# liuzuxin/FSRL

Measured on NVIDIA H100. Metric: env-steps/sec (collect+update) SafetyCarCircle-v0 PPO-Lag, higher is better.
Workload: dtype f32

## Files before the change

### fsrl_b200/csrc/ppo_persist.cu

```cuda
#include "ppo_persist.cuh"
#include "arena.cuh"
#include "ppo_loss.cuh"
#include "wgmma.cuh"
#include <cstdlib>
#include <cmath>
#include <vector>

namespace fsrl {
namespace pp {

using namespace wg;

constexpr int WQ = 2;
constexpr int NEPI = 128 * WQ;
constexpr int TPB = NEPI + 32;
constexpr int C1 = 16 / WQ;
constexpr int C2 = 32 / WQ;
constexpr int RB = 64;
constexpr int MB = 256;
constexpr int KC = 32, NCH = 256 / KC;
constexpr int SLOT_BYTES = 32768, NSLOT = 4;
constexpr int A_CHUNK = 64 * KC * 4;
constexpr int ACC_LD = 68;
constexpr int OUTP = 8;
constexpr int H_ = 256;
constexpr int IMG = 65536;
enum { I_H1A_HI, I_H1A_LO, I_H1T_HI, I_H1T_LO, I_DZA_HI, I_DZA_LO, I_DZT_HI, I_DZT_LO, I_W2A_HI, I_W2A_LO, I_W2B_HI, I_W2B_LO, N_IMG };
constexpr int DB2P_OFF = N_IMG * IMG;
constexpr int DW3P_OFF = DB2P_OFF + 4 * H_;
constexpr int DB3P_OFF = DW3P_OFF + 4 * H_ * OUTP;
constexpr int MAXD = 40;
constexpr int NSMAX = (MAXD + 1) * 32 + 32 + 32 * OUTP + 16;
constexpr int SLICE_OFF = DB3P_OFF + 4 * 16;
constexpr int NET_WS = SLICE_OFF + 8 * NSMAX;
constexpr int SUMSQ_FLOATS = 128;
constexpr int FLAG_LINE = 32;
constexpr int F_A = 0, F_C = 1, F_PER_NET = 2;
constexpr int TILE_PK = (64 * 64 / NEPI + 2) / 3;
constexpr int TILE_FLOATS = TILE_PK * NEPI * 4;
constexpr int SLICE_PK = (NSMAX + 2) / 3;
constexpr int XG_PER_NET = 16 * TILE_FLOATS + 8 * SLICE_PK * 4;
constexpr int MAX_MB = 16384;
constexpr long long WAIT_CYCLES = 6000000000LL;

struct Args {
    fsrl_ppo_update_t u;
    int n_mb, slot0;
    long long adam_t0;
    float* ws;
    unsigned* flags;
    int* err;
    const float* adam_tab;
    long long* dbg;
    int dbg_step;
    unsigned dp_seq;
    int dp_direct;
};
constexpr int DBG_CH = 48;
constexpr int DBG_N = DBG_CH + 2 * 3 * NCH;
#define STAMP(i) do { if (P.dbg && t == P.dbg_step) P.dbg[(size_t)blockIdx.x * DBG_N + (i)] = clock64(); } while (0)

struct AdamS { float w1, b2, w2, rbc2s, eps, neg_step; };
__device__ __forceinline__ float adam_one(float p, float g, float& m, float& v, const AdamS& a) {
    m = m + a.w1 * (g - m);
    v = v * a.b2 + (a.w2 * g) * g;
    const float sq = v > 0.f ? v * rsqrtf(v) : 0.f;
    const float denom = fmaf(sq, a.rbc2s, a.eps);
    return p + __fdividef(a.neg_step * m, denom);
}

__device__ __forceinline__ void fail(int* err, int code) {
    *reinterpret_cast<volatile int*>(err) = code;
    __threadfence_system();
    asm volatile("trap;");
}
__device__ __forceinline__ uint32_t pk_hash(float x, float y, float z) {
    const uint32_t a = __float_as_uint(x), b = __float_as_uint(y), c = __float_as_uint(z);
    return a ^ __funnelshift_l(b, b, 11) ^ __funnelshift_l(c, c, 22);
}
__device__ __forceinline__ bool pk_ok(const float4& v, uint32_t tag) { return (__float_as_uint(v.w) ^ pk_hash(v.x, v.y, v.z)) == tag; }
__device__ __forceinline__ void st_packet(float* p, float x, float y, float z, uint32_t tag) {
    asm volatile("st.relaxed.sys.global.v4.f32 [%0], {%1,%2,%3,%4};" ::"l"(p), "f"(x), "f"(y), "f"(z), "f"(__uint_as_float(tag ^ pk_hash(x, y, z))) : "memory");
}
__device__ __forceinline__ float4 ld_packet(const float* p) {
    float4 v;
    asm volatile("ld.relaxed.sys.global.v4.f32 {%0,%1,%2,%3}, [%4];" : "=f"(v.x), "=f"(v.y), "=f"(v.z), "=f"(v.w) : "l"(p) : "memory");
    return v;
}

__device__ __noinline__ float3 dp_gather(const float* src, long long stride, int me, int world, uint32_t tag,
                                        float ox, float oy, float oz, int* err, int code) {
    const long long t0w = clock64();
    float ax = 0.f, ay = 0.f, az = 0.f;
    for (int r0 = 0; r0 < world; r0 += 4) {
        float4 v[4];
        bool ok;
        do {
            ok = true;
#pragma unroll
            for (int k = 0; k < 4; ++k)
                if (r0 + k < world && r0 + k != me) v[k] = ld_packet(src + (size_t)(r0 + k) * stride);
#pragma unroll
            for (int k = 0; k < 4; ++k)
                if (r0 + k < world && r0 + k != me) ok = ok && pk_ok(v[k], tag);
            if (!ok && clock64() - t0w > 4 * WAIT_CYCLES) fail(err, code);
        } while (!ok);
#pragma unroll
        for (int k = 0; k < 4; ++k) {
            if (r0 + k >= world) continue;
            if (r0 + k == me) { ax += ox; ay += oy; az += oz; }
            else { ax += v[k].x; ay += v[k].y; az += v[k].z; }
        }
    }
    return make_float3(ax, ay, az);
}
__device__ __noinline__ void dp_push_all(const float* const* xg, size_t off, int me, int world, float x, float y, float z, uint32_t tag) {
    for (int r = 0; r < world; ++r)
        if (r != me) st_packet(const_cast<float*>(xg[r]) + off, x, y, z, tag);
}

__device__ __forceinline__ uint32_t mapa_u32(uint32_t local_saddr, uint32_t rank) {
    uint32_t r;
    asm volatile("mapa.shared::cluster.u32 %0, %1, %2;" : "=r"(r) : "r"(local_saddr), "r"(rank));
    return r;
}
__device__ __forceinline__ void st_cluster4(uint32_t raddr, float4 v) {
    asm volatile("st.shared::cluster.v4.f32 [%0], {%1,%2,%3,%4};" ::"r"(raddr), "f"(v.x), "f"(v.y), "f"(v.z), "f"(v.w) : "memory");
}
__device__ __forceinline__ void st_async4(uint32_t raddr, float4 v, uint32_t rbar) {
    asm volatile("st.async.weak.shared::cluster.mbarrier::complete_tx::bytes.v4.f32 [%0], {%1,%2,%3,%4}, [%5];"
                 ::"r"(raddr), "f"(v.x), "f"(v.y), "f"(v.z), "f"(v.w), "r"(rbar) : "memory");
}
__device__ __forceinline__ float ld_cluster(uint32_t raddr) {
    float v;
    asm volatile("ld.shared::cluster.f32 %0, [%1];" : "=f"(v) : "r"(raddr) : "memory");
    return v;
}
__device__ __forceinline__ void mbar_arrive_release_cluster2(uint32_t raddr0, uint32_t raddr1) {
    asm volatile("fence.acq_rel.cluster;\n\t"
                 "mbarrier.arrive.relaxed.cluster.shared::cluster.b64 _, [%0];\n\t"
                 "mbarrier.arrive.relaxed.cluster.shared::cluster.b64 _, [%1];" ::"r"(raddr0), "r"(raddr1) : "memory");
}
__device__ __forceinline__ bool mbar_wait_cluster(uint64_t* bar, uint32_t parity, long long timeout_cycles) {
    const long long t0 = clock64();
    while (true) {
        uint32_t ok;
        asm volatile(
            "{\n\t.reg .pred p;\n\t"
            "mbarrier.try_wait.parity.acquire.cluster.shared::cta.b64 p, [%1], %2;\n\t"
            "selp.u32 %0, 1, 0, p;\n\t}"
            : "=r"(ok) : "r"(smem_u32(bar)), "r"(parity) : "memory");
        if (ok) return true;
        if (clock64() - t0 > timeout_cycles) return false;
    }
}
__device__ __forceinline__ void cluster_sync_all() {
    asm volatile("barrier.cluster.arrive.release.aligned;\n\tbarrier.cluster.wait.acquire.aligned;" ::: "memory");
}

__device__ __forceinline__ bool elect_one() {
    uint32_t pred = 0;
    asm volatile(
        "{\n\t.reg .b32 rx;\n\t.reg .pred px;\n\t"
        "elect.sync rx|px, 0xffffffff;\n\t"
        "selp.u32 %0, 1, 0, px;\n\t}"
        : "=r"(pred));
    return pred != 0;
}
__device__ __forceinline__ void epi_bar() { asm volatile("bar.sync 1, %0;" ::"n"(NEPI) : "memory"); }
__device__ __forceinline__ void prefetch_l2(const void* p) { asm volatile("prefetch.global.L2 [%0];" ::"l"(p)); }

template <int NC>
__device__ __forceinline__ void acc_ld(const float* accs, int row, int col, float (&v)[NC]) {
#pragma unroll
    for (int q = 0; q < NC / 4; ++q) {
        const float4 x = *reinterpret_cast<const float4*>(accs + row * ACC_LD + col + 4 * q);
        v[4 * q] = x.x; v[4 * q + 1] = x.y; v[4 * q + 2] = x.z; v[4 * q + 3] = x.w;
    }
}
template <int NC>
__device__ __forceinline__ void acc_st(float* accs, int row, int col, const float (&v)[NC]) {
#pragma unroll
    for (int q = 0; q < NC / 4; ++q)
        *reinterpret_cast<float4*>(accs + row * ACC_LD + col + 4 * q) = make_float4(v[4 * q], v[4 * q + 1], v[4 * q + 2], v[4 * q + 3]);
}

template <int N>
__device__ __forceinline__ void gemm_phase(const unsigned char* ring, unsigned& qq, uint64_t* bar_full, uint32_t empty_r,
                                           float (&dm)[N / 2], float (&dc)[N / 2], int* err, int code, int lane,
                                           const Args& P, int t, int g) {
#pragma unroll
    for (int e = 0; e < N / 2; ++e) dm[e] = dc[e] = 0.f;
    const uint32_t ring_a = smem_u32(ring);
    constexpr uint32_t b_lbo = 16 * N, b_chunk = N * KC * 4;
    for (int j = 0; j < NCH; ++j, ++qq) {
        const int s = qq % NSLOT;
        if (!mbar_wait(&bar_full[s], (qq / NSLOT) & 1, WAIT_CYCLES)) fail(err, code);
#ifdef FSRL_PPO_CHUNK_STAMPS
        if (P.dbg && t == P.dbg_step && threadIdx.x < 32) P.dbg[(size_t)blockIdx.x * DBG_N + DBG_CH + 3 * NCH * g + 2 * NCH + j] = clock64();
#endif
        __syncwarp();
        wgmma_fence();
        const uint32_t base = ring_a + (uint32_t)s * SLOT_BYTES;
        const uint64_t ah0 = smem_desc(base, 1024, 128), al0 = smem_desc(base + A_CHUNK, 1024, 128);
        const uint64_t bh0 = smem_desc(base + 2 * A_CHUNK, b_lbo, 128), bl0 = smem_desc(base + 2 * A_CHUNK + b_chunk, b_lbo, 128);
#pragma unroll
        for (int ks = 0; ks < KC / 8; ++ks) {
            const uint64_t ah = ah0 + ks * (2048 / 16), al = al0 + ks * (2048 / 16);
            const uint64_t bh = bh0 + ks * (2 * b_lbo / 16), bl = bl0 + ks * (2 * b_lbo / 16);
            if constexpr (N == 32) {
                mma_m64n32k8_tf32(dc, al, bh);
                mma_m64n32k8_tf32(dc, ah, bl);
                mma_m64n32k8_tf32(dm, ah, bh);
            } else {
                mma_m64n64k8_tf32(dc, al, bh);
                mma_m64n64k8_tf32(dc, ah, bl);
                mma_m64n64k8_tf32(dm, ah, bh);
            }
        }
        wgmma_commit();
        if (j > 0) {
            wgmma_wait<1>();
            __syncwarp();
            if (lane < 8) mbar_arrive_cluster(empty_r + 8 * ((qq - 1) % NSLOT));
        }
    }
    wgmma_wait<0>();
    reg_fence(dm); reg_fence(dc);
    __syncwarp();
    if (lane < 8) mbar_arrive_cluster(empty_r + 8 * ((qq - 1) % NSLOT));
}
template <int N>
__device__ __forceinline__ void stage_acc(float* accs, const float (&dm)[N / 2], const float (&dc)[N / 2], int wq, int sp,
                                          int lane) {
    if (wq == 0) {
        const int r = 16 * sp + (lane >> 2);
#pragma unroll
        for (int i = 0; i < N / 8; ++i) {
            const int c = 8 * i + 2 * (lane & 3);
            *reinterpret_cast<float2*>(accs + r * ACC_LD + c) = make_float2(dm[4 * i] + dc[4 * i], dm[4 * i + 1] + dc[4 * i + 1]);
            *reinterpret_cast<float2*>(accs + (r + 8) * ACC_LD + c) =
                make_float2(dm[4 * i + 2] + dc[4 * i + 2], dm[4 * i + 3] + dc[4 * i + 3]);
        }
    }
    asm volatile("bar.sync %0, 64;" ::"r"(2 + sp) : "memory");
}

__device__ __forceinline__ void copy_operand(unsigned char* dst, const float* src, uint32_t bytes, uint64_t* bar, int g, int i,
                                             uint16_t cta_mask) {
    if (g == 1) {
        bulk_g2s(dst, src, bytes, bar);
        bulk_g2s(dst + bytes, src + IMG, bytes, bar);
        return;
    }
    const uint32_t piece = 2 * bytes / g, off = i * piece, part = off / bytes, in = off % bytes;
    bulk_g2s_multicast(dst + off, src + (size_t)part * IMG + in / 4, piece, bar, cta_mask);
}

template <int NC, int W>
__device__ __forceinline__ void transposed_stage(float* scr, const float (&hi)[NC], const float (&lo)[NC], int row, int c0) {
    constexpr int LO = W * 65;
#pragma unroll
    for (int j = 0; j < NC; ++j) {
        scr[(c0 + j) * 65 + row] = hi[j];
        scr[LO + (c0 + j) * 65 + row] = lo[j];
    }
}
template <int W>
__device__ __forceinline__ void transposed_flush(const float* scr, int et, float* img_hi, int row_base, int col_base) {
    constexpr int LO = W * 65;
    const int col = et % W;
    constexpr int GPT = 16 / (NEPI / W);
    const int g0 = (et / W) * GPT;
    float* dst = img_hi + (size_t)(row_base >> 2) * 256 + (size_t)(col_base + col) * 4;
#pragma unroll
    for (int q = 0; q < GPT; ++q) {
        const int g = g0 + q;
        const float* sh = scr + col * 65 + 4 * g;
        *reinterpret_cast<float4*>(dst + (size_t)g * 256) = make_float4(sh[0], sh[1], sh[2], sh[3]);
        *reinterpret_cast<float4*>(dst + IMG + (size_t)g * 256) = make_float4(sh[LO], sh[LO + 1], sh[LO + 2], sh[LO + 3]);
    }
}
template <int NC, int W>
__device__ __forceinline__ void store_transposed(float* scr, const float (&hi)[NC], const float (&lo)[NC], int row, int c0,
                                                 int et, float* img_hi, int row_base, int col_base) {
    transposed_stage<NC, W>(scr, hi, lo, row, c0);
    epi_bar();
    transposed_flush<W>(scr, et, img_hi, row_base, col_base);
    epi_bar();
}

__device__ __forceinline__ float half_sum(float v) {
#pragma unroll
    for (int o = 8; o > 0; o >>= 1) v += __shfl_xor_sync(0xffffffffu, v, o);
    return v;
}

struct SliceMap {
    int w1, b2, w3, b3, n;
    __device__ __host__ SliceMap(int D) { w1 = 0; b2 = (D + 1) * 32; w3 = b2 + 32; b3 = w3 + 32 * OUTP; n = b3 + 16; }
};

struct DpCtx {
    const float* const* xg;
    long long region;
    int me, world;
    uint32_t tag;
    int* err;
    int direct;
};
__device__ __forceinline__ int dp_owner(int et, int q, int world) { return (int)((unsigned)((et >> 5) * TILE_PK + q) % (unsigned)world); }

__device__ __noinline__ void dp_tile_send(DpCtx d, size_t off, const float* accs, int trow, int cb2, int et) {
    float g[C2];
    acc_ld<C2>(accs, trow, cb2, g);
#pragma unroll
    for (int q = 0; q < TILE_PK; ++q) {
        const size_t o_q = (size_t)d.me * d.region + off + (size_t)q * NEPI * 4;
        const float x = g[3 * q], y = 3 * q + 1 < C2 ? g[3 * q + 1] : 0.f, z = 3 * q + 2 < C2 ? g[3 * q + 2] : 0.f;
        if (d.direct) {
            dp_push_all(d.xg, o_q, d.me, d.world, x, y, z, d.tag);
        } else {
            const int o = dp_owner(et, q, d.world);
            if (o != d.me) st_packet(const_cast<float*>(d.xg[o]) + o_q, x, y, z, d.tag);
        }
    }
}
__device__ __noinline__ void dp_tile_reduce(DpCtx d, size_t off, float* accs, int trow, int cb2, int et) {
    float g[C2];
    acc_ld<C2>(accs, trow, cb2, g);
    const float inv_world = 1.0f / (float)d.world;
    const float* loc = d.xg[d.me];
#pragma unroll
    for (int q = 0; q < TILE_PK; ++q) {
        if (dp_owner(et, q, d.world) != d.me) continue;
        const float3 s3 = dp_gather(loc + off + (size_t)q * NEPI * 4, d.region, d.me, d.world, d.tag, g[3 * q],
                                    3 * q + 1 < C2 ? g[3 * q + 1] : 0.f, 3 * q + 2 < C2 ? g[3 * q + 2] : 0.f, d.err, 41);
        const float ax = s3.x * inv_world, ay = s3.y * inv_world, az = s3.z * inv_world;
        dp_push_all(d.xg, (size_t)FSRL_P2P_MAX_RANKS * d.region + off + (size_t)q * NEPI * 4, d.me, d.world, ax, ay, az, d.tag);
        g[3 * q] = ax;
        if (3 * q + 1 < C2) g[3 * q + 1] = ay;
        if (3 * q + 2 < C2) g[3 * q + 2] = az;
    }
    acc_st<C2>(accs, trow, cb2, g);
}
__device__ __noinline__ float dp_tile_finish(DpCtx d, size_t off, float* accs, int trow, int cb2, int et) {
    float g[C2];
    const long long t0w = clock64();
    if (d.direct) {
        float own[C2];
        acc_ld<C2>(accs, trow, cb2, own);
#pragma unroll
        for (int jq = 0; jq < C2; ++jq) g[jq] = 0.f;
        for (int r = 0; r < d.world; ++r) {
            if (r == d.me) {
#pragma unroll
                for (int jq = 0; jq < C2; ++jq) g[jq] += own[jq];
                continue;
            }
            const float* src = d.xg[d.me] + (size_t)r * d.region + off;
            float4 v[TILE_PK];
            bool ok;
            do {
                ok = true;
#pragma unroll
                for (int q = 0; q < TILE_PK; ++q) v[q] = ld_packet(src + (size_t)q * NEPI * 4);
#pragma unroll
                for (int q = 0; q < TILE_PK; ++q) ok = ok && pk_ok(v[q], d.tag);
                if (!ok && clock64() - t0w > 4 * WAIT_CYCLES) fail(d.err, 42);
            } while (!ok);
#pragma unroll
            for (int q = 0; q < TILE_PK; ++q) {
// ... 44 lines not shown
                    sp_g[3 * i], 3 * i + 1 < n ? sp_g[3 * i + 1] : 0.f, 3 * i + 2 < n ? sp_g[3 * i + 2] : 0.f, d.tag);
    const float* loc = d.xg[d.me];
    for (int i = et; i < n3; i += NEPI) {
        const float3 s3 = dp_gather(loc + off_s + 4 * (size_t)i, d.region, d.me, d.world, d.tag, sp_g[3 * i],
                                    3 * i + 1 < n ? sp_g[3 * i + 1] : 0.f, 3 * i + 2 < n ? sp_g[3 * i + 2] : 0.f, d.err, 40);
        sp_g[3 * i] = s3.x * inv_world;
        if (3 * i + 1 < n) sp_g[3 * i + 1] = s3.y * inv_world;
        if (3 * i + 2 < n) sp_g[3 * i + 2] = s3.z * inv_world;
    }
}

__device__ __forceinline__ bool red_cta() { return ((blockIdx.x >> 3) & 3) == ((blockIdx.x & 7) >> 2); }

__device__ __noinline__ float dp_tail(DpCtx d, size_t off_t, size_t off_s, float* accs, float* sp_g, int n, int trow, int cb2,
                                      int et, bool tile, bool slice) {
    if (tile && !d.direct) dp_tile_reduce(d, off_t, accs, trow, cb2, et);
    if (slice) dp_slices(d, off_s, sp_g, n, et);
    __syncwarp();
    return tile ? dp_tile_finish(d, off_t, accs, trow, cb2, et) : 0.f;
}

template <bool DP>
__global__ void __launch_bounds__(TPB, 1) ppo_persist_kernel(const Args P) {
    extern __shared__ __align__(1024) unsigned char smem_raw[];
    __shared__ __align__(8) uint64_t bar_full[NSLOT], bar_empty[NSLOT], bar_b, bar_w1;
    __shared__ float s_red[4][320];
    __shared__ float s_misc[32];
    __shared__ AdamS s_adam;
    __shared__ const float* s_xg[2][FSRL_P2P_MAX_RANKS];
    const fsrl_ppo_update_t& u = P.u;
    const int tid = threadIdx.x, warp = tid >> 5, lane = tid & 31;
    const int net = blockIdx.x >> 5, c = blockIdx.x & 31, a = c >> 3, b = c & 7;
    const bool is_g2 = c < 16;
    const int ka = (c & 15) >> 2, q4 = c & 3;

    const int D = u.D, A = u.A, C = u.C, H = H_;
    const int out = (net == 0) ? A : 1;
    const int n_cta = 32 * u.n_nets;
    float* wsn = P.ws + (size_t)net * NET_WS;
    float* sumsq_g = P.ws + (size_t)u.n_nets * NET_WS;
    unsigned* fl_net = P.flags + (size_t)net * F_PER_NET * FLAG_LINE;
    unsigned* fl_d2 = P.flags + (size_t)u.n_nets * F_PER_NET * FLAG_LINE;
    unsigned char* ring = smem_raw;
    float* accs = reinterpret_cast<float*>(smem_raw + NSLOT * SLOT_BYTES);
    float* small = accs + 64 * ACC_LD;
    const SliceMap sm(D);
    float* sp_p = small;
    float* sp_m = small + sm.n;
    float* sp_v = small + 2 * sm.n;
    float* sp_g = small + 3 * sm.n;
    float* land = small + 4 * sm.n;

    if (tid == 0) {
        for (int i = 0; i < NSLOT; ++i) { mbar_init(&bar_full[i], 1); mbar_init(&bar_empty[i], 4 * 8); }
        mbar_init(&bar_b, 1);
        mbar_init(&bar_w1, 4);
        fence_mbar_init();
    }
    __syncthreads();
    if (DP && threadIdx.x < 2 * FSRL_P2P_MAX_RANKS) s_xg[threadIdx.x / FSRL_P2P_MAX_RANKS][threadIdx.x % FSRL_P2P_MAX_RANKS] = P.u.p2p_xg[threadIdx.x / FSRL_P2P_MAX_RANKS][threadIdx.x % FSRL_P2P_MAX_RANKS];
    if (DP) __syncthreads();
    cluster_sync_all();

    const long long pbase = u.net_off[net];
    const ArenaLayout L = arena_layout(D, H, out, 0);
    const long long o_w1 = pbase + L.w1, o_b1 = pbase + L.b1, o_w2 = pbase + L.w2, o_b2 = pbase + L.b2,
                    o_w3 = pbase + L.w3, o_b3 = pbase + L.b3, o_ls = pbase + L.extra;

    if (warp == NEPI / 32) {
        if (elect_one()) {
            unsigned qq = 0;
            for (int t = 0; t < P.n_mb; ++t) {
                if (!flag_wait_ge<true>(fl_net + F_A * FLAG_LINE, 32u * (t + 1), WAIT_CYCLES)) fail(P.err, 10);
                STAMP(12);
                fence_proxy_async_global();
#pragma unroll 1
                for (int j = 0; j < NCH; ++j, ++qq) {
                    const int s = qq % NSLOT;
                    if (!mbar_wait(&bar_empty[s], ((qq / NSLOT) & 1) ^ 1, WAIT_CYCLES)) fail(P.err, 11);
#ifdef FSRL_PPO_CHUNK_STAMPS
                    STAMP(DBG_CH + j);
#endif
                    unsigned char* dst = ring + (size_t)s * SLOT_BYTES;
                    mbar_expect_tx(&bar_full[s], 3 * A_CHUNK);
                    const size_t ao = (size_t)a * 16384 + (size_t)j * 64 * KC, bo = (size_t)b * 8192 + (size_t)j * 32 * KC;
                    copy_operand(dst, wsn + (size_t)I_H1A_HI * IMG + ao, A_CHUNK, &bar_full[s], 8, b, 0xff);
                    copy_operand(dst + 2 * A_CHUNK, wsn + (size_t)I_W2A_HI * IMG + bo, A_CHUNK / 2, &bar_full[s], 1, 0, 0);
#ifdef FSRL_PPO_CHUNK_STAMPS
                    STAMP(DBG_CH + NCH + j);
#endif
                }
                STAMP(13);
                if (!flag_wait_ge<true>(fl_net + F_C * FLAG_LINE, 32u * (t + 1), WAIT_CYCLES)) fail(P.err, 12);
                STAMP(14);
                fence_proxy_async_global();
                const int ia = is_g2 ? I_W2B_HI : I_DZT_HI, ib = is_g2 ? I_DZA_HI : I_H1T_HI;
                const int blk_a = is_g2 ? ka : q4, blk_b = is_g2 ? q4 : ka;
                const uint16_t m4 = (uint16_t)(0xfu << (b & 4)), m2 = (uint16_t)(0x11u << (b & 3));
#pragma unroll 1
                for (int j = 0; j < NCH; ++j, ++qq) {
                    const int s = qq % NSLOT;
                    if (!mbar_wait(&bar_empty[s], ((qq / NSLOT) & 1) ^ 1, WAIT_CYCLES)) fail(P.err, 13);
#ifdef FSRL_PPO_CHUNK_STAMPS
                    STAMP(DBG_CH + 3 * NCH + j);
#endif
                    unsigned char* dst = ring + (size_t)s * SLOT_BYTES;
                    mbar_expect_tx(&bar_full[s], 4 * A_CHUNK);
                    const size_t ao = (size_t)blk_a * 16384 + (size_t)j * 64 * KC, bo = (size_t)blk_b * 16384 + (size_t)j * 64 * KC;
                    copy_operand(dst, wsn + (size_t)ia * IMG + ao, A_CHUNK, &bar_full[s], is_g2 ? 4 : 2, is_g2 ? b & 3 : b >> 2, is_g2 ? m4 : m2);
                    copy_operand(dst + 2 * A_CHUNK, wsn + (size_t)ib * IMG + bo, A_CHUNK, &bar_full[s], is_g2 ? 2 : 4, is_g2 ? b >> 2 : b & 3, is_g2 ? m2 : m4);
#ifdef FSRL_PPO_CHUNK_STAMPS
                    STAMP(DBG_CH + 4 * NCH + j);
#endif
                }
            }
        }
    } else {
        const int et = tid;
        const int sp = warp & 3;
        const int wq = warp >> 2;
        const int r16 = lane & 15, half = lane >> 4;
        const int trow = 16 * sp + r16;
        const int cb1 = 16 * half + C1 * wq;
        const int cb2 = 32 * half + C2 * wq;
        unsigned qq = 0;
        const uint32_t empty_r = mapa_u32(smem_u32(bar_empty), lane < 8 ? lane : 0);
        float w2p[C2], w2m[C2], w2v[C2];
        const int world = DP ? u.world : 1;
        auto dp_ctx = [&](int t_) {
            DpCtx d;
            const unsigned long long id = (unsigned long long)(P.adam_t0 + t_ + 1);
            d.xg = s_xg[(int)(id & 1ULL)];
            d.region = (long long)u.n_nets * XG_PER_NET;
            d.me = u.p2p_rank; d.world = world;
            d.tag = (P.dp_seq << 16) | (uint32_t)((t_ + 1) & 0xffff);
            d.err = P.err;
            d.direct = P.dp_direct;
            return d;
        };

        for (int i = et; i < sm.n; i += NEPI) {
            long long src = -1;
            if (i < sm.b2) { const int d = i / 32, kk = i % 32; src = (d < D) ? o_w1 + (long long)d * H + 32 * b + kk : o_b1 + 32 * b + kk; }
            else if (i < sm.w3) src = o_b2 + 32 * b + (i - sm.b2);
            else if (i < sm.b3) { const int oo = (i - sm.w3) / OUTP, jj = (i - sm.w3) % OUTP; if (jj < out) src = o_w3 + (long long)(32 * b + oo) * out + jj; }
            else { const int jj = i - sm.b3; if (jj < out) src = o_b3 + jj; else if (net == 0 && jj >= 8 && jj < 8 + A) src = o_ls + (jj - 8); }
            sp_p[i] = src >= 0 ? u.theta[src] : 0.f;
            sp_m[i] = src >= 0 ? u.adam_m[src] : 0.f;
            sp_v[i] = src >= 0 ? u.adam_v[src] : 0.f;
            sp_g[i] = 0.f;
        }
        if (!is_g2) {
            const int o = 64 * q4 + trow;
#pragma unroll
            for (int j = 0; j < C2; ++j) {
                const long long idx = o_w2 + (long long)(64 * ka + cb2 + j) * H + o;
                w2p[j] = u.theta[idx]; w2m[j] = u.adam_m[idx]; w2v[j] = u.adam_v[idx];
            }
        } else {
#pragma unroll
            for (int j = 0; j < C2; ++j) w2p[j] = w2m[j] = w2v[j] = 0.f;
        }
        epi_bar();

        for (int t = 0; t < P.n_mb; ++t) {
            const long long row0 = (long long)t * MB;
            const int slot = P.slot0 + t;
            if (et == 0) {
                s_adam.w1 = (float)(1.0 - u.beta1); s_adam.b2 = (float)u.beta2; s_adam.w2 = (float)(1.0 - u.beta2);
                s_adam.rbc2s = __ldg(P.adam_tab + 2 * t); s_adam.eps = (float)u.adam_eps; s_adam.neg_step = __ldg(P.adam_tab + 2 * t + 1);
                STAMP(0);
                if (P.dbg && t == P.dbg_step) { long long gt; asm volatile("mov.u64 %0, %%globaltimer;" : "=l"(gt)); P.dbg[(size_t)blockIdx.x * DBG_N + 30] = gt; }
                if (P.dbg && t == P.dbg_step + 64) {
                    long long gt; asm volatile("mov.u64 %0, %%globaltimer;" : "=l"(gt));
                    P.dbg[(size_t)blockIdx.x * DBG_N + 31] = gt;
                    P.dbg[(size_t)blockIdx.x * DBG_N + 29] = clock64();
                }
            }
            if (t + 1 < P.n_mb && et < 64) {
                const long long r = row0 + MB + 64 * a + et;
                prefetch_l2(u.obs + r * D);
                if (D > 32) prefetch_l2(u.obs + r * D + 32);
                if (is_g2) { prefetch_l2(u.obs + (r + 128) * D); if (D > 32) prefetch_l2(u.obs + (r + 128) * D + 32); }
                if (net == 0) { prefetch_l2(u.act + r * A); prefetch_l2(u.logp_old + r); prefetch_l2(u.adv + r); if (C > 1) prefetch_l2(u.adv + u.ld + r); }
                else { prefetch_l2(u.ret + (long long)(net - 1) * u.ld + r); if (u.value_clip) prefetch_l2(u.values + (long long)(net - 1) * u.ld + r); }
            }
            float* scratch = reinterpret_cast<float*>(ring);
            if (!is_g2) {
                const float (&pv)[C2] = w2p;
                float phi[C2], plo[C2];
                const int o = 64 * q4 + trow;
                float* w2a_hi = wsn + (size_t)I_W2A_HI * IMG + (size_t)(o >> 5) * 8192 + (size_t)(o & 31) * 4;
                float* w2a_lo = w2a_hi + IMG;
#pragma unroll
                for (int q = 0; q < C2 / 4; ++q) {
                    float4 hi, lo;
                    tf32_split(pv[4 * q], hi.x, lo.x); tf32_split(pv[4 * q + 1], hi.y, lo.y);
                    tf32_split(pv[4 * q + 2], hi.z, lo.z); tf32_split(pv[4 * q + 3], hi.w, lo.w);
                    const size_t plane = (size_t)(16 * ka + (cb2 >> 2) + q) * 128;
                    *reinterpret_cast<float4*>(w2a_hi + plane) = hi;
                    *reinterpret_cast<float4*>(w2a_lo + plane) = lo;
                    phi[4 * q] = hi.x; phi[4 * q + 1] = hi.y; phi[4 * q + 2] = hi.z; phi[4 * q + 3] = hi.w;
                    plo[4 * q] = lo.x; plo[4 * q + 1] = lo.y; plo[4 * q + 2] = lo.z; plo[4 * q + 3] = lo.w;
                }
                store_transposed<C2, 64>(scratch, phi, plo, trow, cb2, et, wsn + (size_t)I_W2B_HI * IMG + (size_t)ka * 16384, 64 * q4, 0);
            }
            if (is_g2) {
                const int r = et & 63, kc = C1 * (et >> 6);
                const float* x0 = u.obs + (row0 + 64 * a + r) * D;
                const float* x1 = u.obs + (row0 + 64 * (a + 2) + r) * D;
                float acc2[2][C1];
#pragma unroll
                for (int j = 0; j < C1; ++j) acc2[0][j] = acc2[1][j] = sp_p[sm.w1 + D * 32 + kc + j];
                for (int d = 0; d < D; ++d) {
                    const float xv0 = __ldg(x0 + d), xv1 = __ldg(x1 + d);
                    const float* w = sp_p + sm.w1 + d * 32 + kc;
#pragma unroll
                    for (int j = 0; j < C1; ++j) { acc2[0][j] = fmaf(xv0, w[j], acc2[0][j]); acc2[1][j] = fmaf(xv1, w[j], acc2[1][j]); }
                }
                constexpr int TSCR = 2 * 32 * 65;
#pragma unroll
                for (int rep = 0; rep < 2; ++rep) {
                    const int aa = a + 2 * rep;
                    float hi[C1], lo[C1];
                    float* a_hi = wsn + (size_t)I_H1A_HI * IMG + (size_t)aa * 16384 + (size_t)r * 4;
#pragma unroll
                    for (int q = 0; q < C1 / 4; ++q) {
#pragma unroll
                        for (int e = 0; e < 4; ++e) tf32_split(fmaxf(acc2[rep][4 * q + e], 0.f), hi[4 * q + e], lo[4 * q + e]);
                        const size_t plane = (size_t)(8 * b + (kc >> 2) + q) * 256;
                        *reinterpret_cast<float4*>(a_hi + plane) = make_float4(hi[4 * q], hi[4 * q + 1], hi[4 * q + 2], hi[4 * q + 3]);
                        *reinterpret_cast<float4*>(a_hi + IMG + plane) = make_float4(lo[4 * q], lo[4 * q + 1], lo[4 * q + 2], lo[4 * q + 3]);
                    }
                    transposed_stage<C1, 32>(scratch + rep * TSCR, hi, lo, r, kc);
                }
                epi_bar();
#pragma unroll
                for (int rep = 0; rep < 2; ++rep)
                    transposed_flush<32>(scratch + rep * TSCR, et, wsn + (size_t)I_H1T_HI * IMG + (size_t)(b >> 1) * 16384, 64 * (a + 2 * rep), 32 * (b & 1));
            }
            fence_proxy_async_smem();
            epi_bar();
            if (et == 0) { STAMP(1); flag_add_release(fl_net + F_A * FLAG_LINE); }

            const long long grow = row0 + 64 * a + trow;
            float p_act[8], p_lpo = 0.f, p_adv0 = 0.f, p_adv1 = 0.f, p_ret = 0.f, p_val = 0.f, mean[2] = {0.f, 0.f}, rstd[2] = {1.f, 1.f};
#pragma unroll
            for (int j = 0; j < 8; ++j) p_act[j] = 0.f;
            if (net == 0) {
#pragma unroll
                for (int j = 0; j < 8; ++j) if (j < A) p_act[j] = __ldg(u.act + grow * A + j);
                p_lpo = __ldg(u.logp_old + grow);
                p_adv0 = __ldg(u.adv + grow);
                if (C > 1) p_adv1 = __ldg(u.adv + u.ld + grow);
                const float* ms = u.mb_stats + (size_t)t * 4;
                mean[0] = __ldg(ms); rstd[0] = __ldg(ms + 1); mean[1] = __ldg(ms + 2); rstd[1] = __ldg(ms + 3);
            } else {
                p_ret = __ldg(u.ret + (long long)(net - 1) * u.ld + grow);
                if (u.value_clip) p_val = __ldg(u.values + (long long)(net - 1) * u.ld + grow);
            }
            float p_ls[8], p_rsg[8];
#pragma unroll
            for (int j = 0; j < 8; ++j) {
                p_ls[j] = (net == 0 && j < A) ? sp_p[sm.b3 + 8 + j] : 0.f;
                p_rsg[j] = 1.0f / expf(p_ls[j]);
            }

            {
                float dm[16], dc[16];
                if (wq == 0) gemm_phase<32>(ring, qq, bar_full, empty_r, dm, dc, P.err, 30, lane, P, t, 0);
                else qq += NCH;
                stage_acc<32>(accs, dm, dc, wq, sp, lane);
            }
            if (et == 0) STAMP(2);
            float h2[C1];
            acc_ld<C1>(accs, trow, cb1, h2);
            float hp[OUTP];
#pragma unroll
            for (int j = 0; j < OUTP; ++j) hp[j] = 0.f;
#pragma unroll
            for (int j = 0; j < C1; ++j) {
                h2[j] = fmaxf(h2[j] + sp_p[sm.b2 + cb1 + j], 0.f);
                const float* w = sp_p + sm.w3 + (cb1 + j) * OUTP;
#pragma unroll
                for (int jj = 0; jj < OUTP; ++jj) hp[jj] = fmaf(h2[j], w[jj], hp[jj]);
            }
#pragma unroll
            for (int jj = 0; jj < OUTP; ++jj) hp[jj] += __shfl_xor_sync(0xffffffffu, hp[jj], 16);
            if (WQ > 1) {
                float* xh = &s_red[0][0];
                if (half == 0 && wq > 0) {
#pragma unroll
                    for (int jj = 0; jj < OUTP; ++jj) xh[((wq - 1) * 64 + trow) * OUTP + jj] = hp[jj];
                }
                epi_bar();
                if (half == 0 && wq == 0) {
#pragma unroll
                    for (int w2 = 1; w2 < WQ; ++w2)
// ... 59 lines not shown
            {
                float hi[C1], lo[C1];
                float* a_hi = wsn + (size_t)I_DZA_HI * IMG + (size_t)a * 16384 + (size_t)trow * 4;
#pragma unroll
                for (int q = 0; q < C1 / 4; ++q) {
#pragma unroll
                    for (int e = 0; e < 4; ++e) tf32_split(dz[4 * q + e], hi[4 * q + e], lo[4 * q + e]);
                    const size_t plane = (size_t)(8 * b + (cb1 >> 2) + q) * 256;
                    *reinterpret_cast<float4*>(a_hi + plane) = make_float4(hi[4 * q], hi[4 * q + 1], hi[4 * q + 2], hi[4 * q + 3]);
                    *reinterpret_cast<float4*>(a_hi + IMG + plane) = make_float4(lo[4 * q], lo[4 * q + 1], lo[4 * q + 2], lo[4 * q + 3]);
                }
                store_transposed<C1, 32>(scratch, hi, lo, trow, cb1, et, wsn + (size_t)I_DZT_HI * IMG + (size_t)(b >> 1) * 16384, 64 * a, 32 * (b & 1));
            }
            if (et == 0) STAMP(27);
            {
                float* row = &s_red[sp][0];
#pragma unroll
                for (int j = 0; j < C1; ++j) {
                    const float sdz = half_sum(dz[j]);
                    if (r16 == 0) row[cb1 + j] = sdz;
                }
#pragma unroll
                for (int jj = 0; jj < OUTP; ++jj) {
                    if (jj < nfeed) {
#pragma unroll
                        for (int j = 0; j < C1; ++j) {
                            const float sv = half_sum(h2[j] * dd[jj]);
                            if (r16 == 0) row[32 + 32 * jj + cb1 + j] = sv;
                        }
                    }
                }
                if (b == 0 && wq == 0) {
#pragma unroll
                    for (int j = 0; j < 16; ++j) {
                        const float sv = half_sum(dd[j]);
                        if (lane == 0) row[288 + j] = sv;
                    }
                    const float sa = half_sum(st_a), sb = half_sum(st_b), sc = half_sum(st_c), sdv = half_sum(st_d);
                    if (lane == 0) { row[304] = sa; row[305] = sb; row[306] = sc; row[307] = sdv; }
                }
            }
            epi_bar();
            if (et == 0) STAMP(28);
            for (int i = et; i < 32 + 32 * nfeed; i += NEPI) {
                const float tot = ((s_red[0][i] + s_red[1][i]) + s_red[2][i]) + s_red[3][i];
                if (i < 32) wsn[DB2P_OFF + a * H + 32 * b + i] = tot;
                else wsn[DW3P_OFF + ((size_t)a * H + 32 * b + ((i - 32) & 31)) * OUTP + ((i - 32) >> 5)] = tot;
            }
            if (b == 0) {
                if (et < 20) {
                    const int i = 288 + et;
                    const float tot = ((s_red[0][i] + s_red[1][i]) + s_red[2][i]) + s_red[3][i];
                    if (et < 16) wsn[DB3P_OFF + a * 16 + et] = tot;
                    else {
                        float* stat = u.stats + (size_t)slot * FSRL_PPO_STATS;
                        if (net == 0) { if (et == 16) atomicAdd(stat + ST_ACTOR_REW, tot); if (et == 17) atomicAdd(stat + ST_ACTOR_SAFETY, tot); if (et == 18) atomicAdd(stat + ST_KL, tot); }
                        else if (et == 19) atomicAdd(stat + ST_VF0 + (net - 1), tot);
                    }
                }
                if (net == 0 && a == 0 && et == 20) u.stats[(size_t)slot * FSRL_PPO_STATS + ST_ENTROPY] = ppo_entropy(sp_p + sm.b3 + 8, A);
            }
            fence_proxy_async_smem();
            epi_bar();
            if (et == 0) { STAMP(5); flag_add_release(fl_net + F_C * FLAG_LINE); }

            unsigned mbits = 0;
            if (is_g2) {
                const int k = 64 * ka + trow;
                const float* msk = wsn + (size_t)I_H1A_HI * IMG + (size_t)q4 * 16384 + (size_t)(k >> 2) * 256 + (k & 3);
                float mreg[C2];
#pragma unroll
                for (int jq = 0; jq < C2; ++jq) mreg[jq] = __ldcg(msk + (size_t)(cb2 + jq) * 4);
                float xr[(64 * MAXD + NEPI - 1) / NEPI];
                const int nx = (64 * D + NEPI - 1) / NEPI;
                const float* xb = u.obs + (row0 + 64 * q4) * D;
#pragma unroll
                for (int q = 0; q < (64 * MAXD + NEPI - 1) / NEPI; ++q)
                    xr[q] = (q < nx && et + q * NEPI < 64 * D) ? __ldg(xb + et + q * NEPI) : 0.f;
#pragma unroll
                for (int jq = 0; jq < C2; ++jq) mbits |= (mreg[jq] > 0.f ? 1u : 0u) << jq;
#pragma unroll
                for (int q = 0; q < (64 * MAXD + NEPI - 1) / NEPI; ++q) {
                    const int e = et + q * NEPI;
                    if (q < nx && e < 64 * D) { const int r = e / D; land[e + (r >> 5)] = xr[q]; }
                }
            }
            if (red_cta() && wq == 1) {
                const int tw = et - 128;
                if (tw == 0) {
                    if (!flag_wait_ge(fl_net + F_C * FLAG_LINE, 32u * (t + 1), WAIT_CYCLES)) fail(P.err, 35);
                    STAMP(15);
                }
                asm volatile("bar.sync 6, 128;" ::: "memory");
                for (int i0 = sm.b2 + tw; i0 < sm.n; i0 += 4 * 128) {
                    float pv[4][4];
#pragma unroll
                    for (int e = 0; e < 4; ++e) {
                        const int i = i0 + e * 128;
                        const float* src = wsn;
                        size_t stride = 0;
                        bool real = false;
                        if (i < sm.n) {
                            if (i < sm.w3) { src = wsn + DB2P_OFF + 32 * b + (i - sm.b2); stride = H; real = true; }
                            else if (i < sm.b3) {
                                const int oo = (i - sm.w3) / OUTP, jj = (i - sm.w3) % OUTP;
                                real = jj < out;
                                src = wsn + DW3P_OFF + ((size_t)32 * b + oo) * OUTP + jj; stride = (size_t)H * OUTP;
                            } else {
                                const int jj = i - sm.b3;
                                real = (jj < out) || (net == 0 && jj >= 8 && jj < 8 + A);
                                src = wsn + DB3P_OFF + jj; stride = 16;
                            }
                        }
#pragma unroll
                        for (int q = 0; q < 4; ++q) pv[e][q] = real ? __ldcg(src + q * stride) : 0.f;
                    }
#pragma unroll
                    for (int e = 0; e < 4; ++e) {
                        const int i = i0 + e * 128;
                        if (i < sm.n) {
                            float gsum = 0.f;
#pragma unroll
                            for (int q = 0; q < 4; ++q) gsum += pv[e][q];
                            sp_g[i] = gsum;
                        }
                    }
                }
                if (tw == 0) STAMP(16);
            }
            {
                float dm[32], dc[32];
                if (wq == 0) gemm_phase<64>(ring, qq, bar_full, empty_r, dm, dc, P.err, 32, lane, P, t, 1);
                else qq += NCH;
                stage_acc<64>(accs, dm, dc, wq, sp, lane);
            }
            if (et == 0) STAMP(6);
            float sq = 0.f;
            if (is_g2) {
                float v[C2];
                acc_ld<C2>(accs, trow, cb2, v);
#pragma unroll
                for (int jq = 0; jq < C2; ++jq) v[jq] = ((mbits >> jq) & 1u) ? v[jq] : 0.f;
                epi_bar();
                if (et == 0) STAMP(22);
                const float* xh = land + (size_t)cb2 * D + half;
                float* dst = reinterpret_cast<float*>(ring) + (size_t)wq * (D + 1) * 64 + trow;
                for (int d = 0; d < D; ++d) {
                    float sacc = 0.f;
#pragma unroll
                    for (int jq = 0; jq < C2; ++jq) sacc = fmaf(xh[jq * D + d], v[jq], sacc);
                    sacc += __shfl_xor_sync(0xffffffffu, sacc, 16);
                    if (half == 0) dst[d * 64] = sacc;
                }
                float sb1 = 0.f;
#pragma unroll
                for (int jq = 0; jq < C2; ++jq) sb1 += v[jq];
                sb1 += __shfl_xor_sync(0xffffffffu, sb1, 16);
                if (half == 0) dst[D * 64] = sb1;
                if (et == 0) STAMP(23);
                epi_bar();
                if (et == 0) mbar_arrive_release_cluster2(mapa_u32(smem_u32(&bar_w1), 2 * ka), mapa_u32(smem_u32(&bar_w1), 2 * ka + 1));
            } else {
                float g[C2];
                acc_ld<C2>(accs, trow, cb2, g);
                if (DP) {
                    dp_tile_send(dp_ctx(t), (size_t)(net * 16 + (c - 16)) * TILE_FLOATS + (size_t)et * 4, accs, trow, cb2, et);
                    if (et == 0) STAMP(32);
                } else {
#pragma unroll
                    for (int jq = 0; jq < C2; ++jq) sq = fmaf(g[jq], g[jq], sq);
                }
            }
            if (et == 0) STAMP(7);
            if (red_cta()) {
                if (!mbar_wait_cluster(&bar_w1, t & 1, WAIT_CYCLES)) fail(P.err, 33);
                if (et == 0) STAMP(8);
                const uint32_t ring_s = smem_u32(ring);
                const int kb = 32 * (b & 1);
                for (int i0 = et; i0 < sm.b2; i0 += 2 * NEPI) {
                    float pv[2][4 * WQ];
#pragma unroll
                    for (int e = 0; e < 2; ++e) {
                        const int i = i0 + e * NEPI;
                        const uint32_t off = 4u * (uint32_t)((i / 32) * 64 + kb + (i % 32));
#pragma unroll
                        for (int rb = 0; rb < 4; ++rb) {
                            const uint32_t src = mapa_u32(ring_s + off, (uint32_t)((4 * (b >> 1) + rb) & 7));
#pragma unroll
                            for (int w = 0; w < WQ; ++w)
                                pv[e][WQ * rb + w] = i < sm.b2 ? ld_cluster(src + 4u * (uint32_t)(w * (D + 1) * 64)) : 0.f;
                        }
                    }
#pragma unroll
                    for (int e = 0; e < 2; ++e) {
                        const int i = i0 + e * NEPI;
                        if (i < sm.b2) {
                            float gsum = 0.f;
#pragma unroll
                            for (int q = 0; q < 4 * WQ; ++q) gsum += pv[e][q];
                            sp_g[i] = gsum;
                        }
                    }
                }
                epi_bar();
                if (et == 0) STAMP(17);
            }
            if (DP) {
                const DpCtx d = dp_ctx(t);
                const size_t off_t = (size_t)(net * 16 + (c - 16)) * TILE_FLOATS + (size_t)et * 4;
                sq += dp_tail(d, off_t, (size_t)u.n_nets * 16 * TILE_FLOATS + (size_t)(net * 8 + b) * SLICE_PK * 4, accs, sp_g, sm.n,
                              trow, cb2, et, !is_g2, red_cta());
                if (et == 0) STAMP(41);
                epi_bar();
            }
            if (red_cta()) {
                for (int i = et; i < sm.n; i += NEPI) {
                    bool real = true;
                    if (i >= sm.w3 && i < sm.b3) real = ((i - sm.w3) % OUTP) < out;
                    else if (i >= sm.b3) { const int jj = i - sm.b3; real = (jj < out) || (net == 0 && jj >= 8 && jj < 8 + A); }
                    if (real && (i < sm.b3 || b == 0)) sq = fmaf(sp_g[i], sp_g[i], sq);
                    wsn[SLICE_OFF + (size_t)b * NSMAX + i] = sp_g[i];
                }
            }
            if (red_cta() || !is_g2) {
                sq = warp_sum(sq);
                if (lane == 0) s_misc[warp] = sq;
                epi_bar();
                if (et == 0) {
                    float tot = 0.f;
#pragma unroll
                    for (int w2 = 0; w2 < NEPI / 32; ++w2) tot += s_misc[w2];
                    sumsq_g[blockIdx.x - (red_cta() ? 8 * a : 0)] = tot;
                    STAMP(9);
                    flag_add_release(fl_d2);
                }
            }
            if (et == 0) {
                if (!flag_wait_ge(fl_d2, 24u * (unsigned)u.n_nets * (t + 1), WAIT_CYCLES)) fail(P.err, 34);
                STAMP(10);
            }
            epi_bar();
            float nq[4];
#pragma unroll
            for (int q = 0; q < 4; ++q) nq[q] = (lane + 32 * q < n_cta) ? __ldcg(sumsq_g + lane + 32 * q) : 0.f;
            if (!DP && !red_cta())
                for (int i = et; i < sm.n; i += NEPI) sp_g[i] = __ldcg(wsn + SLICE_OFF + (size_t)b * NSMAX + i);
            float nsq = ((nq[0] + nq[1]) + nq[2]) + nq[3];
            nsq = warp_sum(nsq);
            float gscale = 1.0f;
            if (u.max_grad_norm > 0.f) gscale = fminf(u.max_grad_norm / (sqrtf(nsq) + 1e-6f), 1.0f);
            if (blockIdx.x == 0 && et == 0) u.stats[(size_t)slot * FSRL_PPO_STATS + ST_GRADNORM] = sqrtf(nsq);
            const AdamS ad = s_adam;
            if (et == 0) STAMP(24);
            for (int i = et; i < sm.n; i += NEPI) {
                float m = sp_m[i], v = sp_v[i];
                const float g = (DP && !red_cta()) ? __ldcg(wsn + SLICE_OFF + (size_t)b * NSMAX + i) : sp_g[i];
                sp_p[i] = adam_one(sp_p[i], g * gscale, m, v, ad);
                sp_m[i] = m; sp_v[i] = v;
            }
            if (et == 0) STAMP(25);
            if (!is_g2) {
                float g[C2];
                acc_ld<C2>(accs, trow, cb2, g);
#pragma unroll
                for (int j = 0; j < C2; ++j) w2p[j] = adam_one(w2p[j], g[j] * gscale, w2m[j], w2v[j], ad);
            }
            epi_bar();
            if (et == 0) STAMP(11);
        }

        if (a == 0) {
            for (int i = et; i < sm.n; i += NEPI) {
                long long dst = -1;
                if (i < sm.b2) { const int d = i / 32, kk = i % 32; dst = (d < D) ? o_w1 + (long long)d * H + 32 * b + kk : o_b1 + 32 * b + kk; }
                else if (i < sm.w3) dst = o_b2 + 32 * b + (i - sm.b2);
                else if (i < sm.b3) { const int oo = (i - sm.w3) / OUTP, jj = (i - sm.w3) % OUTP; if (jj < out) dst = o_w3 + (long long)(32 * b + oo) * out + jj; }
                else if (b == 0) { const int jj = i - sm.b3; if (jj < out) dst = o_b3 + jj; else if (net == 0 && jj >= 8 && jj < 8 + A) dst = o_ls + (jj - 8); }
                if (dst >= 0) { u.theta[dst] = sp_p[i]; u.adam_m[dst] = sp_m[i]; u.adam_v[dst] = sp_v[i]; }
            }
        }
        if (!is_g2) {
            const int o = 64 * q4 + trow;
#pragma unroll
            for (int j = 0; j < C2; ++j) {
                const long long idx = o_w2 + (long long)(64 * ka + cb2 + j) * H + o;
                u.theta[idx] = w2p[j]; u.adam_m[idx] = w2m[j]; u.adam_v[idx] = w2v[j];
            }
        }
    }
    __syncthreads();
    cluster_sync_all();
}

static size_t smem_bytes(int D) {
    return (size_t)NSLOT * SLOT_BYTES + sizeof(float) * 64 * ACC_LD + 4 * sizeof(float) * SliceMap(D).n +
           sizeof(float) * 8 * 64 * OUTP;
}

static cudaLaunchConfig_t cluster_launch(int n_nets, size_t smem, cudaStream_t s, cudaLaunchAttribute* at) {
    at->id = cudaLaunchAttributeClusterDimension;
    at->val.clusterDim.x = 8; at->val.clusterDim.y = 1; at->val.clusterDim.z = 1;
    cudaLaunchConfig_t cfg = {};
    cfg.gridDim = dim3(32 * n_nets); cfg.blockDim = dim3(TPB); cfg.dynamicSmemBytes = smem; cfg.stream = s;
    cfg.attrs = at; cfg.numAttrs = 1;
    return cfg;
}

struct Instance {
    void (*kern)(const Args);
    int max_clusters;
};
static const Instance& instance(bool dp) {
    static Instance inst[2] = {};
    Instance& in = inst[dp];
    if (!in.kern) {
        in.kern = dp ? ppo_persist_kernel<true> : ppo_persist_kernel<false>;
        cudaLaunchAttribute at;
        const cudaLaunchConfig_t cfg = cluster_launch(1, smem_bytes(MAXD), nullptr, &at);
        if (cudaFuncSetAttribute(in.kern, cudaFuncAttributeMaxDynamicSharedMemorySize, (int)cfg.dynamicSmemBytes) != cudaSuccess ||
            cudaOccupancyMaxActiveClusters(&in.max_clusters, in.kern, &cfg) != cudaSuccess) {
            cudaGetLastError();
            in.max_clusters = 0;
        }
    }
    return in;
}

}

size_t ppo_persist_ws_floats(int n_nets, int D, int H) {
    (void)D; (void)H;
    return (size_t)n_nets * pp::NET_WS + pp::SUMSQ_FLOATS + (size_t)(n_nets * pp::F_PER_NET + 1) * pp::FLAG_LINE + 32 +
           2 * (size_t)pp::MAX_MB + 2 * (size_t)32 * n_nets * pp::DBG_N;
}

size_t ppo_persist_p2p_floats(int n_nets) { return (size_t)(FSRL_P2P_MAX_RANKS + 1) * n_nets * pp::XG_PER_NET + 64; }

bool ppo_persist_supported(const fsrl_ppo_update_t& u, long long n_total, int batch_size) {
    if (u.H != 256 || batch_size != pp::MB || n_total % pp::MB != 0 || n_total < pp::MB || n_total / pp::MB > pp::MAX_MB) return false;
    if (u.world > 1 && !(u.p2p_on && u.world <= FSRL_P2P_MAX_RANKS && (size_t)u.p2p_stride >= ppo_persist_p2p_floats(u.n_nets))) return false;
    if (u.D < 1 || u.D > pp::MAXD || u.A > 8 || u.n_nets < 1 || u.n_nets > 3) return false;
    if (u.persist_ws == nullptr || (size_t)u.persist_ws_floats < ppo_persist_ws_floats(u.n_nets, u.D, u.H)) return false;
    if (32 * u.n_nets > sm_count()) return false;
    return pp::instance(u.world > 1).max_clusters >= 4 * u.n_nets;
}

int ppo_persist_run(const fsrl_ppo_update_t& ug, int n_mb, int stats_slot0, long long adam_t0, cudaStream_t s) {
    pp::Args a;
// ... 38 lines not shown
```

Measured before the change: 2.871 million.

## Merge split-TF32 N=32 GEMM into two N=64 wgmmas via zero-padded W2A layout

Re-lays out the W2A operand image as 96-float planes holding zero, hi and lo parts, so each k-step of the N=32 GEMM becomes two m64n64 wgmmas. Offset B descriptors pick up [hi|lo] and [0|hi]-style column windows, which produces the main and correction accumulators in one register block. That block is split back into dm/dc at the end. This cuts the wgmma instruction count per k-step from three to two and replaces the operand copy with a single bulk copy. The cost is extra zero stores, a larger W2A chunk transfer per ring slot, and a 32-float accumulator array.

```diff
diff --git a/fsrl_b200/csrc/ppo_persist.cu b/fsrl_b200/csrc/ppo_persist.cu
--- a/fsrl_b200/csrc/ppo_persist.cu
+++ b/fsrl_b200/csrc/ppo_persist.cu
@@ -25,7 +25,8 @@
 constexpr int OUTP = 8;
 constexpr int H_ = 256;
 constexpr int IMG = 65536;
-enum { I_H1A_HI, I_H1A_LO, I_H1T_HI, I_H1T_LO, I_DZA_HI, I_DZA_LO, I_DZT_HI, I_DZT_LO, I_W2A_HI, I_W2A_LO, I_W2B_HI, I_W2B_LO, N_IMG };
+constexpr int W2A_PLANE = 96 * 4, W2A_BLOCK = 64 * W2A_PLANE, W2A_CHUNK = 8 * W2A_PLANE * 4;
+enum { I_H1A_HI, I_H1A_LO, I_H1T_HI, I_H1T_LO, I_DZA_HI, I_DZA_LO, I_DZT_HI, I_DZT_LO, I_W2A, I_W2B_HI = I_W2A + 3, I_W2B_LO, N_IMG };
 constexpr int DB2P_OFF = N_IMG * IMG;
 constexpr int DW3P_OFF = DB2P_OFF + 4 * H_;
 constexpr int DB3P_OFF = DW3P_OFF + 4 * H_ * OUTP;
@@ -191,6 +192,9 @@
                                            const Args& P, int t, int g) {
 #pragma unroll
     for (int e = 0; e < N / 2; ++e) dm[e] = dc[e] = 0.f;
+    float w[N == 32 ? 32 : 1];
+#pragma unroll
+    for (int e = 0; e < (N == 32 ? 32 : 1); ++e) w[e] = 0.f;
     const uint32_t ring_a = smem_u32(ring);
     constexpr uint32_t b_lbo = 16 * N, b_chunk = N * KC * 4;
     for (int j = 0; j < NCH; ++j, ++qq) {
@@ -209,9 +213,9 @@
             const uint64_t ah = ah0 + ks * (2048 / 16), al = al0 + ks * (2048 / 16);
             const uint64_t bh = bh0 + ks * (2 * b_lbo / 16), bl = bl0 + ks * (2 * b_lbo / 16);
             if constexpr (N == 32) {
-                mma_m64n32k8_tf32(dc, al, bh);
-                mma_m64n32k8_tf32(dc, ah, bl);
-                mma_m64n32k8_tf32(dm, ah, bh);
+                const uint64_t bz = smem_desc(base + 2 * A_CHUNK, W2A_PLANE * 4, 128) + ks * (2 * W2A_PLANE * 4 / 16);
+                mma_m64n64k8_tf32(w, al, bz);
+                mma_m64n64k8_tf32(w, ah, bz + 512 / 16);
             } else {
                 mma_m64n64k8_tf32(dc, al, bh);
                 mma_m64n64k8_tf32(dc, ah, bl);
@@ -226,6 +230,11 @@
         }
     }
     wgmma_wait<0>();
+    if constexpr (N == 32) {
+        reg_fence(w);
+#pragma unroll
+        for (int e = 0; e < 16; ++e) { dm[e] = w[e]; dc[e] = w[16 + e]; }
+    }
     reg_fence(dm); reg_fence(dc);
     __syncwarp();
     if (lane < 8) mbar_arrive_cluster(empty_r + 8 * ((qq - 1) % NSLOT));
@@ -498,10 +507,10 @@
                     STAMP(DBG_CH + j);
 #endif
                     unsigned char* dst = ring + (size_t)s * SLOT_BYTES;
-                    mbar_expect_tx(&bar_full[s], 3 * A_CHUNK);
-                    const size_t ao = (size_t)a * 16384 + (size_t)j * 64 * KC, bo = (size_t)b * 8192 + (size_t)j * 32 * KC;
+                    mbar_expect_tx(&bar_full[s], 2 * A_CHUNK + W2A_CHUNK);
+                    const size_t ao = (size_t)a * 16384 + (size_t)j * 64 * KC, bo = (size_t)b * W2A_BLOCK + (size_t)j * 8 * W2A_PLANE;
                     copy_operand(dst, wsn + (size_t)I_H1A_HI * IMG + ao, A_CHUNK, &bar_full[s], 8, b, 0xff);
-                    copy_operand(dst + 2 * A_CHUNK, wsn + (size_t)I_W2A_HI * IMG + bo, A_CHUNK / 2, &bar_full[s], 1, 0, 0);
+                    bulk_g2s(dst + 2 * A_CHUNK, wsn + (size_t)I_W2A * IMG + bo, W2A_CHUNK, &bar_full[s]);
 #ifdef FSRL_PPO_CHUNK_STAMPS
                     STAMP(DBG_CH + NCH + j);
 #endif
@@ -606,16 +615,16 @@
                 const float (&pv)[C2] = w2p;
                 float phi[C2], plo[C2];
                 const int o = 64 * q4 + trow;
-                float* w2a_hi = wsn + (size_t)I_W2A_HI * IMG + (size_t)(o >> 5) * 8192 + (size_t)(o & 31) * 4;
-                float* w2a_lo = w2a_hi + IMG;
+                float* w2a_z = wsn + (size_t)I_W2A * IMG + (size_t)(o >> 5) * W2A_BLOCK + (size_t)(o & 31) * 4;
 #pragma unroll
                 for (int q = 0; q < C2 / 4; ++q) {
                     float4 hi, lo;
                     tf32_split(pv[4 * q], hi.x, lo.x); tf32_split(pv[4 * q + 1], hi.y, lo.y);
                     tf32_split(pv[4 * q + 2], hi.z, lo.z); tf32_split(pv[4 * q + 3], hi.w, lo.w);
-                    const size_t plane = (size_t)(16 * ka + (cb2 >> 2) + q) * 128;
-                    *reinterpret_cast<float4*>(w2a_hi + plane) = hi;
-                    *reinterpret_cast<float4*>(w2a_lo + plane) = lo;
+                    float* pl = w2a_z + (size_t)(16 * ka + (cb2 >> 2) + q) * W2A_PLANE;
+                    *reinterpret_cast<float4*>(pl) = make_float4(0.f, 0.f, 0.f, 0.f);
+                    *reinterpret_cast<float4*>(pl + 128) = hi;
+                    *reinterpret_cast<float4*>(pl + 256) = lo;
                     phi[4 * q] = hi.x; phi[4 * q + 1] = hi.y; phi[4 * q + 2] = hi.z; phi[4 * q + 3] = hi.w;
                     plo[4 * q] = lo.x; plo[4 * q + 1] = lo.y; plo[4 * q + 2] = lo.z; plo[4 * q + 3] = lo.w;
                 }
```

Result: no change. 2.846 million, median of 6 (-0.9%).

## Prefetch next minibatch observations into shared memory with async copies; vectorize dW1 reduction

Applied to the files above, without the earlier changes.

The layer-1 forward in the g2 warpgroup now reads observation rows from a shared-memory staging buffer. That buffer is filled with cp.async for the next minibatch while the current step is still in its gradient-norm wait and Adam update, instead of using global __ldg reads on the critical path. The dW1 partial reduction also pads the landed x tile to a multiple of 4 and reads it as float4, computing four outputs per pass. This adds shared-memory aliasing inside the ring (guarded by a static_assert) and extra pipeline waits, which risks hazards if the ring is reused at the same time.

```diff
diff --git a/fsrl_b200/csrc/ppo_persist.cu b/fsrl_b200/csrc/ppo_persist.cu
--- a/fsrl_b200/csrc/ppo_persist.cu
+++ b/fsrl_b200/csrc/ppo_persist.cu
@@ -2,6 +2,7 @@
 #include "arena.cuh"
 #include "ppo_loss.cuh"
 #include "wgmma.cuh"
+#include <cuda_pipeline.h>
 #include <cstdlib>
 #include <cmath>
 #include <vector>
@@ -30,6 +31,9 @@
 constexpr int DW3P_OFF = DB2P_OFF + 4 * H_;
 constexpr int DB3P_OFF = DW3P_OFF + 4 * H_ * OUTP;
 constexpr int MAXD = 40;
+constexpr int XS_OFF = 2 * SLOT_BYTES;
+static_assert(XS_OFF >= 2 * 32 * 65 * 2 * 4 && XS_OFF >= 2 * (MAXD + 1) * 64 * 4 &&
+              XS_OFF + 128 * (MAXD + 1) * 4 <= NSLOT * SLOT_BYTES, "staged rows overlap the ring's scratch or dW1 partials");
 constexpr int NSMAX = (MAXD + 1) * 32 + 32 + 32 * OUTP + 16;
 constexpr int SLICE_OFF = DB3P_OFF + 4 * 16;
 constexpr int NET_WS = SLICE_OFF + 8 * NSMAX;
@@ -288,6 +292,14 @@
     epi_bar();
     transposed_flush<W>(scr, et, img_hi, row_base, col_base);
     epi_bar();
+}
+
+__device__ __forceinline__ void stage_rows(float* xs, const float* obs, long long row0, int a, int D, int et) {
+    const int i = et >> 1;
+    const float* src = obs + (row0 + 64 * a + i + (i & 64)) * D;
+    float* dst = xs + i * (D | 1);
+    for (int d = et & 1; d < D; d += 2) __pipeline_memcpy_async(dst + d, src + d, 4);
+    __pipeline_commit();
 }
 
 __device__ __forceinline__ float half_sum(float v) {
@@ -555,6 +567,8 @@
             return d;
         };
 
+        float* xs = reinterpret_cast<float*>(ring + XS_OFF);
+        if (is_g2) stage_rows(xs, u.obs, 0, a, D, et);
         for (int i = et; i < sm.n; i += NEPI) {
             long long src = -1;
             if (i < sm.b2) { const int d = i / 32, kk = i % 32; src = (d < D) ? o_w1 + (long long)d * H + 32 * b + kk : o_b1 + 32 * b + kk; }
@@ -577,6 +591,7 @@
 #pragma unroll
             for (int j = 0; j < C2; ++j) w2p[j] = w2m[j] = w2v[j] = 0.f;
         }
+        __pipeline_wait_prior(0);
         epi_bar();
 
         for (int t = 0; t < P.n_mb; ++t) {
@@ -623,13 +638,13 @@
             }
             if (is_g2) {
                 const int r = et & 63, kc = C1 * (et >> 6);
-                const float* x0 = u.obs + (row0 + 64 * a + r) * D;
-                const float* x1 = u.obs + (row0 + 64 * (a + 2) + r) * D;
+                const float* x0 = xs + r * (D | 1);
+                const float* x1 = xs + (64 + r) * (D | 1);
                 float acc2[2][C1];
 #pragma unroll
                 for (int j = 0; j < C1; ++j) acc2[0][j] = acc2[1][j] = sp_p[sm.w1 + D * 32 + kc + j];
                 for (int d = 0; d < D; ++d) {
-                    const float xv0 = __ldg(x0 + d), xv1 = __ldg(x1 + d);
+                    const float xv0 = x0[d], xv1 = x1[d];
                     const float* w = sp_p + sm.w1 + d * 32 + kc;
 #pragma unroll
                     for (int j = 0; j < C1; ++j) { acc2[0][j] = fmaf(xv0, w[j], acc2[0][j]); acc2[1][j] = fmaf(xv1, w[j], acc2[1][j]); }
@@ -855,7 +870,7 @@
 #pragma unroll
                 for (int q = 0; q < (64 * MAXD + NEPI - 1) / NEPI; ++q) {
                     const int e = et + q * NEPI;
-                    if (q < nx && e < 64 * D) { const int r = e / D; land[e + (r >> 5)] = xr[q]; }
+                    if (q < nx && e < 64 * D) { const int r = e / D; land[r * ((D + 3) & ~3) + 4 * (r >> 5) + (e - r * D)] = xr[q]; }
                 }
             }
             if (red_cta() && wq == 1) {
@@ -916,14 +931,26 @@
                 for (int jq = 0; jq < C2; ++jq) v[jq] = ((mbits >> jq) & 1u) ? v[jq] : 0.f;
                 epi_bar();
                 if (et == 0) STAMP(22);
-                const float* xh = land + (size_t)cb2 * D + half;
+                const int dp4 = (D + 3) & ~3;
+                const float* xh = land + (size_t)cb2 * dp4 + 4 * half;
                 float* dst = reinterpret_cast<float*>(ring) + (size_t)wq * (D + 1) * 64 + trow;
-                for (int d = 0; d < D; ++d) {
-                    float sacc = 0.f;
-#pragma unroll
-                    for (int jq = 0; jq < C2; ++jq) sacc = fmaf(xh[jq * D + d], v[jq], sacc);
-                    sacc += __shfl_xor_sync(0xffffffffu, sacc, 16);
-                    if (half == 0) dst[d * 64] = sacc;
+                for (int d0 = 0; d0 < D; d0 += 4) {
+                    float sacc[4] = {0.f, 0.f, 0.f, 0.f};
+#pragma unroll
+                    for (int jq = 0; jq < C2; ++jq) {
+                        const float4 x = *reinterpret_cast<const float4*>(xh + jq * dp4 + d0);
+                        sacc[0] = fmaf(x.x, v[jq], sacc[0]);
+                        sacc[1] = fmaf(x.y, v[jq], sacc[1]);
+                        sacc[2] = fmaf(x.z, v[jq], sacc[2]);
+                        sacc[3] = fmaf(x.w, v[jq], sacc[3]);
+                    }
+#pragma unroll
+                    for (int i = 0; i < 4; ++i) sacc[i] += __shfl_xor_sync(0xffffffffu, sacc[i], 16);
+                    if (half == 0) {
+#pragma unroll
+                        for (int i = 0; i < 4; ++i)
+                            if (d0 + i < D) dst[(d0 + i) * 64] = sacc[i];
+                    }
                 }
                 float sb1 = 0.f;
 #pragma unroll
@@ -1008,6 +1035,7 @@
                     flag_add_release(fl_d2);
                 }
             }
+            if (is_g2 && t + 1 < P.n_mb) stage_rows(xs, u.obs, row0 + MB, a, D, et);
             if (et == 0) {
                 if (!flag_wait_ge(fl_d2, 24u * (unsigned)u.n_nets * (t + 1), WAIT_CYCLES)) fail(P.err, 34);
                 STAMP(10);
@@ -1037,6 +1065,9 @@
                 acc_ld<C2>(accs, trow, cb2, g);
 #pragma unroll
                 for (int j = 0; j < C2; ++j) w2p[j] = adam_one(w2p[j], g[j] * gscale, w2m[j], w2v[j], ad);
+            } else {
+                __pipeline_wait_prior(0);
+                if (et == 0) STAMP(18);
             }
             epi_bar();
             if (et == 0) STAMP(11);
```

Result: faster. 2.877 million before, 2.981 million after, median of 6 (+3.6%).
